# z619850002/CVIDS

Hardware: AMD Instinct MI355X
Metric: depth frames/sec integrated + Mvoxel-updates/sec, 640x480 @ 1 cm, 1/2/4/8 GPU (higher is better)
Workload: dtype f32; 1 GPU; 640x480 depth+BGR colour stream (sphere_room, 1 agent), 1 cm voxels, chunk 16^3, InverseTruncator(1), carving 0.05 m, projective TSDF integration + marching cubes every 10 frames; image=640x480, chunk=16, color=True, frames_per_call=10, mesh_every=10, parallelism=1 GPU

## Files before the change

cvids_amd/csrc/chisel_device.h:

```cpp
#pragma once
#include <hip/hip_runtime.h>
#include <stdint.h>

namespace chisel_hip {

constexpr uint64_t KEY_EMPTY = ~0ull;
constexpr uint64_t KEY_TOMB = ~0ull - 1ull;
constexpr int ID_BIAS = 1 << 20;
constexpr int INTEGRATE_MAX_GRID = 4096;
constexpr int INTEGRATE_GRID_CAP = 1 << 19;

__host__ __device__ inline uint64_t pack_id(int x, int y, int z) {
    return (uint64_t)(uint32_t)(x + ID_BIAS) | ((uint64_t)(uint32_t)(y + ID_BIAS) << 21) |
           ((uint64_t)(uint32_t)(z + ID_BIAS) << 42);
}
__host__ __device__ inline void unpack_id(uint64_t k, int &x, int &y, int &z) {
    x = (int)(k & 0x1FFFFF) - ID_BIAS;
    y = (int)((k >> 21) & 0x1FFFFF) - ID_BIAS;
    z = (int)((k >> 42) & 0x1FFFFF) - ID_BIAS;
}
__host__ __device__ inline uint64_t chunk_hash(int x, int y, int z) {
    return ((uint64_t)(int64_t)x * 73856093ull) ^ ((uint64_t)(int64_t)y * 19349663ull) ^
           ((uint64_t)(int64_t)z * 8349279ull);
}
// ... 32 lines not shown
    unsigned *mesh_flag;
    int *mesh_jobs;
    int *mesh_ctl;
    int mesh_jobs_capacity;
};

constexpr int MC_TRIS = 0, MC_GRIDS = 1, MC_OVERFLOW = 2, MC_JOBS = 3, MC_KEPT = 4, MC_CURSORS = 8;
constexpr int MC_BBOX = 136, MC_INTS = MC_BBOX + 8;
constexpr int MC_LATCH = 5;
__device__ inline void bbox_include(int *mesh_ctl, int x, int y, int z) {
    if (!mesh_ctl) return;
    int *b = mesh_ctl + MC_BBOX;
    if (x < b[0]) atomicMin(&b[0], x);
    if (y < b[1]) atomicMin(&b[1], y);
    if (z < b[2]) atomicMin(&b[2], z);
    if (x > b[3]) atomicMax(&b[3], x);
    if (y > b[4]) atomicMax(&b[4], y);
    if (z > b[5]) atomicMax(&b[5], z);
}

constexpr unsigned SUM_POS = 1u, SUM_NEG = 2u, SUM_ANY = 3u;
constexpr size_t SLOT_SUMMARY_PAD = 16;
__device__ inline uint32_t *slot_summary(const MapView &M) { return M.slot_dirty + 2 * (size_t)M.max_chunks + SLOT_SUMMARY_PAD; }

__device__ inline bool mark_slot_dirty(const MapView &M, int slot) {
    if (atomicExch(&M.slot_dirty[slot], 1u) == 0u) {
        const unsigned p = atomicAdd(&M.slot_dirty[2 * (size_t)M.max_chunks], 1u);
        if (p < (unsigned)M.max_chunks) M.slot_dirty[(size_t)M.max_chunks + p] = (unsigned)slot;
        return true;
    }
    return false;
}

constexpr int PYR_L0 = 2, PYR_L1 = 6, PYR_LEVELS = PYR_L1 - PYR_L0 + 1;
struct PyramidView {
    float2 *data;
    int off[PYR_LEVELS];
    int w[PYR_LEVELS];
    int h[PYR_LEVELS];
};

struct CameraParams {
    float R[9];
    float t[3];
    float fx, fy, cx, cy;
    int W, H;
};

constexpr int KMAX = 16;

struct IntegratorParams {
    int trunc_kind;
    float trunc_param;
    float weight;
    int carving;
    float carving_dist;
    float res;
    float half_res;
    float diag;
    float max_depth;
    int n_shards, shard_rank, shard_block;
    int single_chunk;
};

typedef float2 PixelRec;

// ... 184 lines not shown
```

cvids_amd/csrc/chisel_hip.hip:

```cpp
#include "../../include/chisel_hip.h"
#include "../../include/chisel_hip_selftest.h"

#include <hip/hip_runtime.h>
#include <hip/hip_ext.h>
#include <dlfcn.h>

#include <algorithm>
#include <array>
#include <atomic>
#include <chrono>
#include <condition_variable>
#include <functional>
#include <mutex>
#include <thread>
#include <cmath>
#include <cstdlib>
#include <cstdio>
#include <cstring>
#include <fstream>
#include <map>
#include <string>
#include <unordered_map>
#include <set>
#include <unordered_set>
// ... 235 lines not shown
    PinnedBuffer<int> mesh_totals_host;
    PinnedBuffer<int> error_flag_host;
    int mesh_seq = 0;
    PinnedBuffer<JobInfo> mesh_info_host;
    hipStream_t copy_stream = nullptr;
    ShellPlan shell_plan{};
    struct ShellMemory { DeviceBuffer<unsigned long long> jobset; DeviceBuffer<int> my_jobs, ctl, send_items; } shell_mem;
    PinnedBuffer<int> shell_plan_host;
    int64_t shell_send[SHELL_MAX_SHARDS][2] = {}, shell_recv[SHELL_MAX_SHARDS][2] = {};
    int shell_jobs = 0, shell_send_items = 0;
    const unsigned char *ghost_packed = nullptr;
    ShellSegments ghost_segments{};
    int ghost_packed_items = 0;
    hipEvent_t order_events[2] = {nullptr, nullptr};
    int64_t shell_stride = 0;
    unsigned shell_items_grid = 2048;
    const int *shell_abort_dev = nullptr;
    bool shell_fixed_ghosts = false, shell_redrop = false, shell_uncommitted = false;
    std::unordered_set<uint64_t, IdHash> pending_mesh_ids;
    uint64_t pending_version = 1;
    uint32_t dirty_epoch = 0;
    bool dirty_tail_queued = false;
    uint64_t dirty_tail_cursor = 0;
    unsigned dirty_tail_batch = 0;
    PinnedBuffer<int> dirty_tail_host;
    int batch_frames = KMAX;
    uint64_t ghost_bytes = 0;
    bool single_chunk = false;
    int single_id[3] = {0, 0, 0};
    bool mesh_mark_needed = false;
    bool mesh_totals_clean = true;
    int64_t removed_since_recompute = 0;
    int mesh_jobs_hint = 0;
    int mesh_stages = 3;
    bool mesh_detached = false;
    uint64_t topology_epoch = 0;
    MeshBuffers mesh_buf{};
    struct MeshMemory {
        DeviceBuffer<MeshJob> jobs; DeviceBuffer<int> ids; DeviceBuffer<JobInfo> info; DeviceBuffer<TriRec> tris; DeviceBuffer<CubeCorners> corners;
        DeviceBuffer<unsigned> cnt; DeviceBuffer<unsigned long long> job_acc; DeviceBuffer<double> query; DeviceBuffer<float> cube;
    } mesh_mem;
    struct CloudBuffers {
        DeviceBuffer<float> points, colors;
        int64_t capacity = 0;
        DeviceBuffer<char> zeroed;
        size_t zeroed_bytes = 0;
        CloudView view{};
        DeviceBuffer<CloudRay> rays; DeviceBuffer<unsigned> rgb; DeviceBuffer<int> tile_prefix, table_vals, pairs, sorted; DeviceBuffer<uint64_t> listed;
    } cloud;
    bool profiling = false;
    std::vector<ProfEvent> prof_live;
    std::vector<hipEvent_t> event_pool;
    double prof_ms[CHISEL_HIP_NUM_KERNELS] = {};
    int64_t prof_launches[CHISEL_HIP_NUM_KERNELS] = {};
};

namespace {

int sync_all(chisel_hip_map *m) {
    for (int pass = 0; pass < 2; pass++) {
        if (m->aux) HIP_TRY(hipStreamSynchronize(m->aux));
        if (m->aux2) HIP_TRY(hipStreamSynchronize(m->aux2));
        if (m->aux3) HIP_TRY(hipStreamSynchronize(m->aux3));
        if (!pass) HIP_TRY(hipStreamSynchronize(m->stream));
    }
    m->complete_seq = m->launch_seq;
// ... 2425 lines not shown
```

cvids_amd/csrc/host_mesh.h:

```cpp
namespace {

MeshParams mesh_params(const chisel_hip_map *m) {
    MeshParams P;
    P.res = m->cfg.voxel_resolution;
    P.half_res = m->cfg.voxel_resolution * 0.5f;
    P.rf_chunk = 1.0f / ((float)m->N * m->cfg.voxel_resolution);
    P.rf_voxel = 1.0f / m->cfg.voxel_resolution;
    P.use_color = m->cfg.use_color ? 1 : 0;
    P.stages = m->mesh_stages & m->tune.mesh_stage_mask;
    return P;
}

void launch_mesh_triangles(chisel_hip_map *m, const MeshParams &P, float *arena, size_t arena_floats, int publish = 0) {
    MeshBuffers &B = m->mesh_buf;
    const JobInfo *bases = B.info;
    const int *totals = B.totals;
    int *host_info = reinterpret_cast<int *>(m->mesh_info_host.dev());
    volatile int *host_flags = (volatile int *)m->mesh_totals_host.dev();
    const int max_jobs = std::min(MESH_INFO_PREFETCH, B.capacity), seq = m->mesh_seq, part = B.tri_capacity / MESH_PARTS;
    const dim3 grid(4096), block(MESH_TRI_BLOCK);
    switch (m->N) {
        case 8: hipLaunchKernelGGL(mesh_triangle_kernel<8>, grid, block, 0, m->stream, m->view, P, B.jobs, bases, B.tris, B.corners, totals, B.cnt, part, arena, arena_floats, host_info, host_flags, max_jobs, seq, publish); break;
        case 16: hipLaunchKernelGGL(mesh_triangle_kernel<16>, grid, block, 0, m->stream, m->view, P, B.jobs, bases, B.tris, B.corners, totals, B.cnt, part, arena, arena_floats, host_info, host_flags, max_jobs, seq, publish); break;
        case 32: hipLaunchKernelGGL(mesh_triangle_kernel<32>, grid, block, 0, m->stream, m->view, P, B.jobs, bases, B.tris, B.corners, totals, B.cnt, part, arena, arena_floats, host_info, host_flags, max_jobs, seq, publish); break;
    }
}

int mesh_subjobs(const chisel_hip_map *m) { return m->N == 8 ? MeshGeom<8>::S : (m->N == 16 ? MeshGeom<16>::S : MeshGeom<32>::S); }
int mesh_row_ints(const chisel_hip_map *m) { return m->N == 8 ? MeshGeom<8>::ROW : (m->N == 16 ? MeshGeom<16>::ROW : MeshGeom<32>::ROW); }
int ensure_mesh_jobs(chisel_hip_map *m, int n) {
    MeshBuffers &B = m->mesh_buf;
    if (n <= B.capacity) return CHISEL_HIP_OK;
    HIP_TRY(hipStreamSynchronize(m->stream));
    chisel_hip_map::MeshMemory &O = m->mesh_mem;
    int cap = std::max(4096, B.capacity);
    while (cap < n) cap *= 2;
    B.capacity = 0;
    HIP_TRY(alloc_viewed(O.jobs, B.jobs, (size_t)cap));
    HIP_TRY(alloc_viewed(O.ids, B.ids, (size_t)cap * 3));
    HIP_TRY(alloc_viewed(O.info, B.info, (size_t)cap));
    HIP_TRY(alloc_viewed(O.cnt, B.cnt, (size_t)cap * mesh_row_ints(m)));
    HIP_TRY(alloc_viewed(O.job_acc, B.job_acc, (size_t)cap));
    HIP_TRY(hipMemsetAsync(B.job_acc, 0, (size_t)cap * sizeof(unsigned long long), m->stream));
    B.capacity = cap;
    return CHISEL_HIP_OK;
}

enum { MT_TRIS = MC_TRIS, MT_GRIDS = MC_GRIDS, MT_OVERFLOW = MC_OVERFLOW, MT_JOBS = MC_JOBS };
int *mesh_totals(chisel_hip_map *m) { return m->mesh_buf.totals; }
hipError_t zero_mesh_counters(chisel_hip_map *m) {
    hipError_t e = hipMemsetAsync(mesh_totals(m), 0, 3 * sizeof(int), m->stream);
    if (e == hipSuccess) e = hipMemsetAsync(mesh_totals(m) + MC_CURSORS, 0, 2 * MESH_PARTS * sizeof(int), m->stream);
    return e;
// ... 107 lines not shown
        case 16: hipLaunchKernelGGL(mesh_count_kernel_16, grid, dim3(64), 0, m->stream, m->view, ids, ids_capacity, B.jobs, n_jobs, B.info, d_totals, B.cnt, B.job_acc, B.tris, B.corners, part, B.flags, keep, done_seq); break;
        case 32: hipLaunchKernelGGL(mesh_count_kernel_32, grid, dim3(64), 0, m->stream, m->view, ids, ids_capacity, B.jobs, n_jobs, B.info, d_totals, B.cnt, B.job_acc, B.tris, B.corners, part, B.flags, keep, done_seq); break;
    }
}

int recompute_meshes(chisel_hip_map *m) {
    RoctxRange range("chisel_hip mesh recompute: count, triangles");
    MeshBuffers &B = m->mesh_buf;
    const MeshParams P = mesh_params(m);
    if (!B.tris) {
        B.tri_capacity = std::max(B.tri_capacity, m->mesh_tiny ? 4 * MESH_PARTS : 1 << 20);
        HIP_TRY(alloc_viewed(m->mesh_mem.tris, B.tris, (size_t)B.tri_capacity));
        HIP_TRY(alloc_viewed(m->mesh_mem.corners, B.corners, (size_t)B.tri_capacity));
    }
    int arena_id = -1;
    for (size_t i = 0; i < m->arenas.size() && arena_id < 0; i++)
        if (!m->arenas[i].dev) arena_id = (int)i;
    if (arena_id < 0) {
        m->arenas.emplace_back();
        arena_id = (int)m->arenas.size() - 1;
    }
    {
        MeshArena &A = m->arenas[arena_id];
        A = MeshArena();
        int rc_a = take_arena_buffer(m, m->mesh_tiny ? (size_t)4096 : std::max<size_t>(2 * m->mesh_need_hint, (size_t)1 << 22), &A.dev, &A.capacity);
        if (rc_a) return rc_a;
    }
    launch_mesh_count(m);
    if (!m->mesh_detached) m->dirty_epoch++;
    m->mesh_seq++;
    m->recomputes++;
    {
        ProfScope ps(m, CHISEL_HIP_KERNEL_MESH);
        launch_mesh_triangles(m, P, m->arenas[arena_id].dev, m->arenas[arena_id].capacity, 1 | (B.n_jobs ? 2 : 0));
    }
    HIP_TRY(hipGetLastError());
    m->pending_meshes.unchecked = true;
    m->pending_meshes.active = false;
    m->pending_meshes.arena = arena_id;
    {
        const size_t want = std::max<size_t>(2 * m->mesh_need_hint, (size_t)1 << 22);
        bool have = false;
        for (const auto &b : m->arena_pool) have = have || b.second >= want;
        if (!have) {
            float *spare = nullptr;
            const size_t cap = want + want / 4 + 1024;
            if (hipMalloc(&spare, cap * sizeof(float)) == hipSuccess) m->arena_pool.emplace_back(spare, cap);
        }
    }
    return CHISEL_HIP_OK;
}

bool mesh_totals_published(const chisel_hip_map *m) { return ((volatile const int *)m->mesh_totals_host.get())[MH_PUBLISHED] == m->mesh_seq; }
int replay_deferred_set(chisel_hip_map *m, int set);
void launch_fixed_drop(chisel_hip_map *m, const int *latch);
int check_mesh_totals(chisel_hip_map *m) {
    if (!m->pending_meshes.unchecked) return CHISEL_HIP_OK;
    m->pending_meshes.unchecked = false;
    const int deferred = m->deferred_set;
    m->deferred_set = -1;
    MeshBuffers &B = m->mesh_buf;
    int *d_totals = mesh_totals(m);
    const bool color = m->cfg.use_color != 0;
    const MeshParams P = mesh_params(m);
    int arena_id = m->pending_meshes.arena;
    {
        volatile int *host = m->mesh_totals_host.get();
// ... 42 lines not shown
                HIP_TRY(hipMemcpyAsync(B.n_jobs, stage, sizeof(int), hipMemcpyHostToDevice, m->stream));
            }
            launch_mesh_count(m);
            if (B.n_jobs) HIP_TRY(hipMemsetAsync(B.n_jobs, 0, sizeof(int), m->stream));
            HIP_TRY(hipMemcpyAsync(totals, d_totals, 4 * sizeof(int), hipMemcpyDeviceToHost, m->stream));
            HIP_TRY(hipStreamSynchronize(m->stream));
            if (!totals[MT_OVERFLOW]) break;
            if (attempt == 12) return fail(CHISEL_HIP_ERR_HIP, "mesh record lists overflow after growing them");
        }
        redo = true;
        HIP_TRY(hipMemcpy(m->mesh_info_host.get(), B.info, (size_t)std::min(MESH_INFO_PREFETCH, B.capacity) * sizeof(JobInfo), hipMemcpyDeviceToHost));
    }
    const int n = totals[MT_JOBS];
    if ((size_t)totals[MT_TRIS] > 0x7fffffffull / 9) return fail(CHISEL_HIP_ERR_UNSUPPORTED, "more than 2^31 / 9 mesh triangles in one recompute");
    const size_t nv = (size_t)totals[MT_TRIS] * 3, ng = (size_t)totals[MT_GRIDS];
    {
        MeshArena &A = m->arenas[arena_id];
        A.nv = nv;
        A.ng = ng;
        A.color = color;
        if (redo ? !device_unfit : (A.floats() > A.capacity) != device_unfit)
            return fail(CHISEL_HIP_ERR_HIP, "mesh recompute: host and device disagree on whether it fitted");
        if (redo || A.floats() > A.capacity) {
            HIP_TRY(hipStreamSynchronize(m->stream));
            HIP_TRY(hipMemsetAsync(mesh_totals(m) + MC_LATCH, 0, sizeof(int), m->stream));
            if (A.floats() > A.capacity) {
                m->arena_pool.emplace_back(A.dev, A.capacity);
                A.dev = nullptr;
                int rc_a = take_arena_buffer(m, A.floats(), &A.dev, &A.capacity);
                if (rc_a) return rc_a;
            }
            {
                ProfScope ps(m, CHISEL_HIP_KERNEL_MESH);
                launch_mesh_triangles(m, P, A.dev, A.capacity);
            }
            HIP_TRY(hipGetLastError());
            latch_guard.settled = true;
            if (m->shell_redrop && m->ghost_packed)
                launch_fixed_drop(m, nullptr);
            if (deferred >= 0) {
                int rc_r = replay_deferred_set(m, deferred);
                if (rc_r) return rc_r;
            }
        }
        m->mesh_need_hint = A.floats();
        if (nv + ng == 0) {
            free_arena(m, A);
            arena_id = -1;
        }
    }
    if (m->shell_redrop) {
        m->shell_redrop = false;
        m->ghost_packed = nullptr;
    }
    m->mesh_jobs_hint = n;
    if (n != 0) {
        m->pending_meshes.active = true;
        m->pending_meshes.n = n;
        m->pending_meshes.arena = arena_id;
    }
    if (pool_error != 0)
        return fail(CHISEL_HIP_ERR_POOL_FULL, pool_error == 1 ? "chunk pool exhausted: raise chisel_hip_config.max_chunks"
                                                              : "chunk hash table exhausted: raise chisel_hip_config.max_chunks");
    return CHISEL_HIP_OK;
}

int resolve_pending_meshes(chisel_hip_map *m) {
    int rc_c = check_mesh_totals(m);
    if (rc_c) return rc_c;
    if (!m->pending_meshes.active) return CHISEL_HIP_OK;
    m->pending_meshes.active = false;
    MeshBuffers &B = m->mesh_buf;
    const int n = m->pending_meshes.n, arena_id = m->pending_meshes.arena;
    {
        volatile int *host = m->mesh_totals_host.get();
        const auto t0 = std::chrono::steady_clock::now();
        while (host[MH_INFO_SEQ] != m->mesh_seq) {
            if (std::chrono::steady_clock::now() - t0 > std::chrono::milliseconds(2)) {
                HIP_TRY(hipStreamSynchronize(m->stream));
                if (host[MH_INFO_SEQ] != m->mesh_seq) return fail(CHISEL_HIP_ERR_HIP, "mesh job records were not published");
            }
        }
        std::atomic_thread_fence(std::memory_order_acquire);
    }
    g_mesh_timer.lap(1);
    std::vector<JobInfo> tail;
    if (n > MESH_INFO_PREFETCH) {
        tail.resize((size_t)n - MESH_INFO_PREFETCH);
// ... 467 lines not shown
```

cvids_amd/csrc/kernels_integrate.h:

```cpp
#pragma once
#include <type_traits>

#include "chisel_device.h"
#include "kernels_cull.h"
#include "kernels_map.h"

namespace chisel_hip {

#ifndef INTEGRATE_WAVES
#define INTEGRATE_WAVES 6
#endif
#ifndef INTEGRATE_BLOCKS_PER_CU
#define INTEGRATE_BLOCKS_PER_CU 6
#endif
#ifndef INTEGRATE_WPB
#define INTEGRATE_WPB 1
#endif
#ifndef INTEGRATE_FINE_BELOW
#define INTEGRATE_FINE_BELOW 600
#endif

#ifndef INTEGRATE_PIPE
#define INTEGRATE_PIPE 0
#endif
// ... 550 lines not shown
            if (!existed) {
                if (bm) {
                    int s = 0;
                    if (lane == 0) s = claim_slot(Mc, sy, cxi, cyi, czi);
                    s = __builtin_amdgcn_readfirstlane(s);
                    const bool created = s >= 0 && (s & CLAIM_CREATED) != 0;
                    slot = s >= 0 ? (s & ~CLAIM_CREATED) : s;
                    n_new += created ? 1u : 0u;
                }
                unsigned seen = 0u;
                if (lane == 0 && bm) seen += atomicOr(&sy->band, bm);
                if (lane < KMAX && carve_v) seen += atomicAdd(&sy->carve[lane], (unsigned)carve_v);
                asm volatile("s_waitcnt vmcnt(0)" : "+v"(seen)::"memory");
                unsigned last = 0u;
                if (lane == 0) last = (atomicAdd(&sy->arrived, 1u) == (unsigned)(G::WPC - 1)) ? 1u : 0u;
                if (__builtin_amdgcn_readfirstlane((int)last)) {
                    unsigned band_all = 0u, cnt = 0u;
                    if (lane == 0) band_all = atomicOr(&sy->band, 0u);
                    if (lane < KMAX) cnt = atomicAdd(&sy->carve[lane], 0u);
                    band_all = (unsigned)__builtin_amdgcn_readfirstlane((int)band_all);
                    const bool counts = band_all != 0u && lane < KMAX && lane > __builtin_ctz(band_all | 0x80000000u);
                    unsigned v = counts ? cnt : 0u;
#pragma unroll
                    for (int o = 8; o > 0; o >>= 1) v += __shfl_down(v, o);
                    if (lane == 0) t_probe += v;
                }
                PHASE(2);
                if (slot < 0) return;
            }
            unsigned signs = 0u;
            {
                const size_t out_base = (size_t)slot * G::V;
                if (st & DCHG) {
                    *reinterpret_cast<QuadF *>((M.sdf + out_base) + lane_off) = s4;
                    *reinterpret_cast<QuadF *>((M.wgt + out_base) + lane_off) = w4;
                }
                if (COLOR && (st & CCHG)) *reinterpret_cast<QuadU *>((M.rgbw + out_base) + lane_off) = c4;
                bool pos = false, neg = false;
#pragma unroll
                for (int j = 0; j < VPL; j++) {
                    const bool seen = (st & DCHG) && f4(w4, j) > 0.5f;
                    neg = neg || (seen && f4(s4, j) < 0.0f);
                    pos = pos || (seen && !(f4(s4, j) < 0.0f));
                }
                signs = (__any(pos) ? SUM_POS : 0u) | (__any(neg) ? SUM_NEG : 0u);
            }
            if (cm) {
                unsigned old = 0u;
                int newly_dirty = 0;
                if (lane == 0) {
                    old = atomicOr(&sy->changed, cm);
                    if (old == 0u) newly_dirty = mark_slot_dirty(M, slot) ? 1 : 0;
                    if (signs) atomicOr(&slot_summary(M)[slot], signs);
                }
                old = (unsigned)__builtin_amdgcn_readfirstlane((int)old);
                n_updated += (unsigned)__popc(cm & ~old);
                if (__builtin_amdgcn_readfirstlane(newly_dirty)) mesh_expand_dirty(Mc, slot, cxi, cyi, czi, lane);
            }
    };
    if (mixed) {
        if (local_unit < units_x) {
            const int u4 = n_coarse_x * G::WPC;
            if (local_unit < u4) run_unit(std::integral_constant<int, VPL0>{}, (local_unit / G::WPC) * 8 + xcd, local_unit % G::WPC, local_unit);
            else run_unit(std::integral_constant<int, 2>{}, (n_coarse_x + (local_unit - u4) / GF::WPC) * 8 + xcd, (local_unit - u4) % GF::WPC, local_unit);
        }
        PHASE(3);
    }
    int wid = mixed ? total : ((local_unit / G::WPC) * 8 + xcd) * G::WPC + local_unit % G::WPC;
    while (wid < total) {
        run_unit(std::integral_constant<int, VPL0>{}, wid / G::WPC, wid % G::WPC, wid);
// ... 94 lines not shown
```

cvids_amd/csrc/kernels_mesh.h:

```cpp
#pragma once
#include "chisel_device.h"
#include "kernels_map.h"
#include "mc_tables.h"

namespace chisel_hip {

__constant__ unsigned long long c_mc_cases[256] = CHISEL_MC_PACKED_CASES;
__constant__ __attribute__((aligned(4))) unsigned char c_mc_counts[256] = CHISEL_MC_VERTEX_COUNTS;
__constant__ unsigned char c_mc_edges[12] = CHISEL_MC_EDGE_CORNERS;

struct MeshJob {
    int x, y, z;
    int nb[27];
    int pad[2];
};
constexpr int NB_SELF = 13;

struct MeshParams {
    float res;
    float half_res;
    float rf_chunk;
    float rf_voxel;
    int use_color;
    int stages;
// ... 225 lines not shown
__device__ inline float fold_corner(float sdf, float weight) { return weight > 0.5f ? sdf : __builtin_nanf(""); }

template <int N>
struct MeshGeom {
    static constexpr int ZL = N == 16 ? 2 : (N == 8 ? 7 : 1);
    static constexpr int NI = (N - 1 + ZL - 1) / ZL;
    static constexpr int S = NI + 3;
    static constexpr int CPL = N == 32 ? 16 : 8;
    static constexpr int MAXC = 64 * CPL;
    static constexpr int TILE = N == 32 ? 33 * 33 * 2 : N * N * (ZL + 1);
    static constexpr int ROW = (2 + S + 3) / 4 * 4;
    static_assert((N - 1) * (N - 1) * ZL <= MAXC && N * N <= MAXC, "cubes per sub-job");
};
template <int N, int TYPE>
struct MeshBox {
    static constexpr int BX = TYPE == 1 ? 1 : (TYPE == 3 ? N : N - 1);
    static constexpr int BY = TYPE == 2 ? 1 : (TYPE == 0 ? N - 1 : N);
    static constexpr int TX = BX + 1, TY = BY + 1;
    static constexpr int X0 = TYPE == 1 ? N - 1 : 0, Y0 = TYPE == 2 ? N - 1 : 0;
    static constexpr unsigned PLUS = TYPE == 0 ? 0x01u : (TYPE == 1 ? 0x0Fu : (TYPE == 2 ? 0x05u : 0xFFu));
};
constexpr int MESH_PARTS = 64;
static_assert(MC_BBOX == MC_CURSORS + 2 * MESH_PARTS, "the created-id box sits behind the cursors");
static_assert(MC_LATCH > MC_KEPT && MC_LATCH < MC_CURSORS, "a free word in front of the cursors");
static_assert(MESH_PARTS == 64, "integrate_kernel zeroes the cursors with one wave");

#ifndef MESH_COUNT_WAVES
#define MESH_COUNT_WAVES 6
#endif
#ifndef MESH_COUNT_VGPRS
#define MESH_COUNT_VGPRS 80
#endif
constexpr int MESH_TRI_BLOCK = 256;
#ifndef MESH_TRI_WAVES
#define MESH_TRI_WAVES 1
#endif

struct JobInfo {
    int x, y, z;
    int present;
    int n_vertices, n_grids;
    int tri_base;
    int grid_base;
};

struct alignas(16) TriRec {
    unsigned job;
    unsigned code;
    unsigned cube;
    unsigned rel;
};
struct alignas(16) CubeCorners {
    float s[8];
};
__device__ inline float pick8(const float (&s)[8], int e) {
    const float a0 = (e & 1) ? s[1] : s[0], a1 = (e & 1) ? s[3] : s[2], a2 = (e & 1) ? s[5] : s[4], a3 = (e & 1) ? s[7] : s[6];
    const float b0 = (e & 2) ? a1 : a0, b1 = (e & 2) ? a3 : a2;
    return (e & 4) ? b1 : b0;
}

#ifdef CHISEL_PHASES
__device__ unsigned long long g_mesh_phase[8];
#define MSTAMP(i) do { if (lane == 0 && (blockIdx.x & 31) == 0) { const unsigned long long n_ = __builtin_amdgcn_s_memrealtime(); atomicAdd(&g_mesh_phase[i], n_ - mt_); mt_ = n_; } } while (0)
#else
#define MSTAMP(i) do { } while (0)
#endif
// ... 33 lines not shown
#endif
        __syncthreads();
        asm volatile("" : "+v"(lane));
        const int jx = ids[3 * j], jy = ids[3 * j + 1], jz = ids[3 * j + 2];
        const int type = s < G::NI ? 0 : s - G::NI + 1;
        const unsigned plus_needed = type == 0 ? MeshBox<N, 0>::PLUS : (type == 1 ? MeshBox<N, 1>::PLUS : (type == 2 ? MeshBox<N, 2>::PLUS : MeshBox<N, 3>::PLUS));
        const int dx = lane % 3 - 1, dy = (lane / 3) % 3 - 1, dz = lane / 9 - 1;
        const bool plus = lane < 27 && dx >= 0 && dy >= 0 && dz >= 0;
        const bool counted = plus && ((plus_needed >> (dx + 2 * dy + 4 * dz)) & 1u);
        int slot = -1;
        unsigned sum = 0u;
        if (lane < 27 && (s == 0 || counted)) slot = hash_find_quiescent(M, jx + dx, jy + dy, jz + dz);
        if (counted && slot >= 0) sum = slot_summary(M)[slot];
        if (lane < 27) s_nb[lane] = slot;
        if (s == 0) {
            if (lane < 27) jobs[j].nb[lane] = slot;
            else if (lane == 27) {
                jobs[j].x = jx;
                jobs[j].y = jy;
                jobs[j].z = jz;
                jobs[j].pad[0] = jobs[j].pad[1] = 0;
            }
        }
        const int self = __shfl(slot, NB_SELF);
        const bool present = self >= 0;
        const bool can = present && (unsigned)__shfl((int)sum, NB_SELF) != 0u && __ballot(counted && (sum & SUM_POS)) != 0ull && __ballot(counted && (sum & SUM_NEG)) != 0ull;
        if (s == 0 && lane == 28 && present && !keep_dirty) {
            if (mesh_flag) mesh_flag[self] = 0u;
            M.slot_dirty[self] = 0u;
        }
        MSTAMP(0);
        auto deposit = [&](int my_nt, int my_ng, int part) -> unsigned long long {
            unsigned long long old = 0ull;
            if (lane == 1) cnt[(size_t)j * G::ROW + 2 + s] = (unsigned)my_nt | ((unsigned)my_ng << 16);
            if (lane == 1 || (lane == 0 && my_ng)) {
                unsigned long long *addr = lane == 0 ? cursors + part : job_acc + j;
                const unsigned long long inc = lane == 0 ? ((unsigned long long)my_ng << 32) | (unsigned long long)my_nt
                                                         : (1ull << 48) | ((unsigned long long)my_ng << 24) | (unsigned long long)my_nt;
                old = atomicAdd(addr, inc);
                if (lane == 1 && (int)(old >> 48) == G::S - 1) {
                    const unsigned long long tot = old + inc;
                    const int tnt = (int)(tot & 0xffffffull), tng = (int)((tot >> 24) & 0xffffffull);
                    unsigned long long base = 0ull;
                    if (tnt | tng) base = atomicAdd(reinterpret_cast<unsigned long long *>(ctl + MC_TRIS), ((unsigned long long)tng << 32) | (unsigned long long)tnt);
                    JobInfo ji;
                    ji.x = jx; ji.y = jy; ji.z = jz;
                    ji.present = present ? 1 : 0;
                    ji.n_vertices = 3 * tnt;
                    ji.n_grids = tng;
                    ji.tri_base = (int)(base & 0xffffffffull);
                    ji.grid_base = (int)(base >> 32);
                    info[j] = ji;
                    cnt[(size_t)j * G::ROW] = (unsigned)ji.tri_base;
                    cnt[(size_t)j * G::ROW + 1] = (unsigned)ji.grid_base;
                    job_acc[j] = 0ull;
                }
            }
            return old;
        };
        if (!can) {
            (void)deposit(0, 0, 0);
            continue;
        }
        auto run = [&](auto type_tag) {
            constexpr int T = decltype(type_tag)::value;
            using B = MeshBox<N, T>;
            const int z0 = T == 0 ? s * G::ZL : (T == 3 ? N - 1 : 0);
            const int bz = T == 0 ? min(G::ZL, N - 1 - z0) : (T == 3 ? 1 : N - 1);
            const int ncubes = B::BX * B::BY * bz;
            if (T == 0) {
                constexpr int PASS = N == 32 ? 4 : ((G::ZL + 1) * N * N / 4 + 63) / 64;
                const int n4 = (bz + 1) * N * N / 4;
                const float4 *sp = reinterpret_cast<const float4 *>(M.sdf + (size_t)self * (N * N * N) + (size_t)z0 * N * N);
                const float4 *wp = reinterpret_cast<const float4 *>(M.wgt + (size_t)self * (N * N * N) + (size_t)z0 * N * N);
                for (int base = 0; base < n4; base += 64 * PASS) {
                    float4 vs[PASS], vw[PASS];
#pragma unroll
                    for (int u = 0; u < PASS; u++) {
                        const int i = min(base + u * 64 + lane, n4 - 1);
                        vs[u] = sp[i];
                        vw[u] = wp[i];
                    }
#pragma unroll
                    for (int u = 0; u < PASS; u++) {
                        const int i = base + u * 64 + lane;
                        if (i < n4)
                            reinterpret_cast<float4 *>(s_tile)[i] = make_float4(fold_corner(vs[u].x, vw[u].x), fold_corner(vs[u].y, vw[u].y),
// ... 69 lines not shown
            }
            const int tv = __shfl(iv, 63), tg = __shfl(ig, 63);
            MSTAMP(3);
            const int part = (j * G::S + s) & (MESH_PARTS - 1);
            const unsigned long long old = deposit(tv / 3, tg, part);
            if (tg == 0) return;
            const unsigned long long cur = (unsigned long long)__shfl((long long)old, 0);
            const int cur_t = (int)(cur & 0xffffffffull), cur_g = (int)(cur >> 32);
            MSTAMP(4);
            if (cur_t + tv / 3 > part_capacity || cur_g + tg > part_capacity) {
                if (lane == 0) ctl[MC_OVERFLOW] = 1;
                return;
            }
            {
                int trel = (iv - nv) / 3, gidx = ig - ng;
#pragma unroll
                for (int k = 0; k < G::CPL; k++) {
                    const int c = lane * G::CPL + k;
                    const int index = (c < ncubes) ? (int)((cw[k >> 2] >> ((k & 3) * 8)) & 0xffu) : 0;
                    if (index == 0) continue;
                    s_list[gidx] = (unsigned)c | ((unsigned)index << 10) | ((unsigned)trel << 18);
                    trel += n_verts(index) / 3;
                    gidx++;
                }
            }
            __syncthreads();
            const size_t base_t = (size_t)part * part_capacity + cur_t, base_g = (size_t)part * part_capacity + cur_g;
            for (int e = lane; e < tg; e += 64) {
                const unsigned a = s_list[e];
                const int c = (int)(a & 1023u), index = (int)((a >> 10) & 255u), trel = (int)(a >> 18);
                CubeCorners cc;
                int idx2;
                (void)cube_corners(c, cc.s, idx2);
                corners[base_g + e] = cc;
                const int x = B::X0 + c % B::BX, y = B::Y0 + (c / B::BX) % B::BY, z = z0 + c / (B::BX * B::BY);
                const int nt = n_verts(index) / 3;
                TriRec rec;
                rec.job = (unsigned)j;
                rec.cube = (unsigned)(base_g + e);
                for (int t = 0; t < nt; t++) {
                    rec.code = (unsigned)x | ((unsigned)y << 5) | ((unsigned)z << 10) | ((unsigned)index << 15) | ((unsigned)t << 23) | ((unsigned)s << 26);
                    rec.rel = (unsigned)(trel + t) | ((unsigned)e << 16);
                    tris[base_t + trel + t] = rec;
                }
            }
            MSTAMP(5);
        };
        switch (type) {
            case 0: run(std::integral_constant<int, 0>()); break;
            case 1: run(std::integral_constant<int, 1>()); break;
            case 2: run(std::integral_constant<int, 2>()); break;
            default: run(std::integral_constant<int, 3>()); break;
        }
    }
}

#define CHISEL_MESH_COUNT_KERNEL(NN, VGPRS, WAVES)                                                                                                    \
    __global__ __launch_bounds__(64, WAVES) __attribute__((amdgpu_num_vgpr(VGPRS))) void mesh_count_kernel_##NN(                                 \
        MapView M, const int *__restrict__ ids, int ids_capacity, MeshJob *jobs, const int *__restrict__ n_jobs, JobInfo *info, int *ctl, unsigned *cnt, \
        unsigned long long *job_acc, TriRec *tris, CubeCorners *corners, int part_capacity, unsigned *mesh_flag, int keep_dirty, int done_seq) { \
        mesh_count_body<NN>(M, ids, ids_capacity, jobs, n_jobs, info, ctl, cnt, job_acc, tris, corners, part_capacity, mesh_flag, keep_dirty, done_seq); \
    }
CHISEL_MESH_COUNT_KERNEL(8, MESH_COUNT_VGPRS, MESH_COUNT_WAVES)
CHISEL_MESH_COUNT_KERNEL(16, MESH_COUNT_VGPRS, MESH_COUNT_WAVES)
CHISEL_MESH_COUNT_KERNEL(32, 128, 3)
#undef CHISEL_MESH_COUNT_KERNEL

__device__ inline f3v interpolate_vertex(f3v v1, f3v v2, float sdf1, float sdf2) {
    const float minDiff = 1e-6;
    const float sdfDiff = sdf1 - sdf2;
    if (fabsf(sdfDiff) < minDiff) return add3(v1, scl3(v2, 0.5f));
    const float t = sdf1 / sdfDiff;
    return add3(v1, scl3(sub3(v2, v1), t));
}

__device__ inline int corner_ox(int i) { return ((i + 1) >> 1) & 1; }
// ... 61 lines not shown
        if (s_off[part + o] <= i) part += o;
    i -= s_off[part];
    TSTAMP(0, i);
    const TriRec rec = tris[(size_t)part * part_capacity + i];
    const MeshJob &job = jobs[rec.job];
    const int *nb = job.nb;
    const int jx = job.x, jy = job.y, jz = job.z;
    const int x = (int)(rec.code & 31u), y = (int)((rec.code >> 5) & 31u), z = (int)((rec.code >> 10) & 31u);
    const int index = (int)((rec.code >> 15) & 0xffu), t = 3 * (int)((rec.code >> 23) & 7u), sub = (int)(rec.code >> 26);
    int tri_pos = (int)(rec.rel & 0xffffu), grid_pos = (int)(rec.rel >> 16);
    {
        const uint4 *row4 = reinterpret_cast<const uint4 *>(cnt + (size_t)rec.job * ROW);
        uint4 r[ROW / 4];
#pragma unroll
        for (int q = 0; q < ROW / 4; q++) r[q] = row4[q];
        tri_pos += (int)r[0].x;
        grid_pos += (int)r[0].y;
#pragma unroll
        for (int q = 2; q < ROW; q++) {
            const unsigned c = (q & 3) == 0 ? r[q >> 2].x : ((q & 3) == 1 ? r[q >> 2].y : ((q & 3) == 2 ? r[q >> 2].z : r[q >> 2].w));
            const unsigned cc = (q - 2 < sub) ? c : 0u;
            tri_pos += (int)(cc & 0xffffu);
            grid_pos += (int)(cc >> 16);
        }
    }
    const int vi = 3 * tri_pos + mine;
    TSTAMP(1, vi);
    const unsigned long long row = c_mc_cases[index];
    const f3v origin = mk3((float)(N * jx) * P.res, (float)(N * jy) * P.res, (float)(N * jz) * P.res);
    const f3v coords = add3(mk3((float)x * P.res + P.half_res, (float)y * P.res + P.half_res, (float)z * P.res + P.half_res), origin);
    const CubeCorners cc = corners[rec.cube];
    if (t == 0 && mine == 0) {
        const size_t g = (size_t)grid_pos;
        grids[3 * g] = coords.x;
        grids[3 * g + 1] = coords.y;
        grids[3 * g + 2] = coords.z;
    }
    f3v p[3];
#pragma unroll
    for (int a = 0; a < 3; a++) {
        const int ed = (int)((row >> (4 * (t + 2 - a))) & 0xF);
        const int e0 = c_mc_edges[ed] & 0xF, e1 = c_mc_edges[ed] >> 4;
        const f3v c0 = add3(coords, mk3((float)corner_ox(e0) * P.res, (float)corner_oy(e0) * P.res, (float)corner_oz(e0) * P.res));
        const f3v c1 = add3(coords, mk3((float)corner_ox(e1) * P.res, (float)corner_oy(e1) * P.res, (float)corner_oz(e1) * P.res));
        const float s0 = pick8(cc.s, e0), s1 = pick8(cc.s, e1);
        p[a] = interpolate_vertex(c0, c1, s0, s1);
    }
    const f3v fn = normalized3(cross3v(sub3(p[1], p[0]), sub3(p[2], p[0])));
    const f3v pv = mine == 0 ? p[0] : (mine == 1 ? p[1] : p[2]);
    float *vo = vertices + 3 * (size_t)vi;
    float *no = normals + 3 * (size_t)vi;
    vo[0] = pv.x;
    vo[1] = pv.y;
    vo[2] = pv.z;
    TSTAMP(2, pv.x);
    f3v nrm = fn;
    double dist;
    f3v grad;
    if ((P.stages & 1) && get_sdf_and_gradient<N>(M, P, pv, jx, jy, jz, nb, dist, grad)) {
        const float mag = sqrtf(sum3f(grad.x * grad.x, grad.y * grad.y, grad.z * grad.z));
        if ((double)mag > 1e-12) nrm = scl3(grad, 1.0f / mag);
    }
    TSTAMP(3, nrm.x);
    no[0] = nrm.x;
    no[1] = nrm.y;
    no[2] = nrm.z;
    if (colors) {
        const f3v col = (P.stages & 2) ? interpolate_color<N>(M, P, pv, jx, jy, jz, nb) : mk3(0.0f, 0.0f, 0.0f);
        float *co = colors + 3 * (size_t)vi;
        TSTAMP(4, col.x);
        co[0] = col.x;
        co[1] = col.y;
        co[2] = col.z;
    }
    }
    }
}

template <int N>
__global__ void mesh_one_cube_kernel(MapView M, MeshParams P, int jx, int jy, int jz, int ix, int iy, int iz, float cx, float cy, float cz, float *out) {
    float sdf[8];
    bool observed = true;
    for (int i = 0; i < 8 && observed; i++) {
        int c[3] = {ix + corner_ox(i), iy + corner_oy(i), iz + corner_oz(i)};
        int off[3] = {0, 0, 0};
        for (int a = 0; a < 3; a++) {
            if (c[a] < 0) { off[a] = -1; c[a] = N - 1; }
            else if (c[a] >= N) { off[a] = 1; c[a] = 0; }
        }
        const int slot = hash_find_quiescent(M, jx + off[0], jy + off[1], jz + off[2]);
        if (slot < 0) { observed = false; break; }
        const size_t o = (size_t)slot * (N * N * N) + (c[2] * N + c[1]) * N + c[0];
        if (!(M.wgt[o] > 0.5f)) { observed = false; break; }
        sdf[i] = M.sdf[o];
    }
    out[0] = 0.0f;
    out[1] = 0.0f;
    if (!observed) return;
    int index = 0;
    for (int i = 0; i < 8; i++) index |= (sdf[i] < 0.0f) ? (1 << i) : 0;
    const int nv = c_mc_counts[index];
    const unsigned long long row = c_mc_cases[index];
    const f3v coords = mk3(cx, cy, cz);
    for (int t = 0; t < nv; t += 3) {
        f3v p[3];
        for (int a = 0; a < 3; a++) {
// ... 121 lines not shown
```

Measured before the change: 106,800 frames/s.

## Size mesh triangle grid from triangle hint and compute face normals lazily

Launches the mesh triangle kernel with a grid sized from the previous triangle count, instead of a fixed 4096 blocks, clamped between 64 and 4096. The per-vertex kernel now interpolates only its own edge vertex and computes the full face normal only when the SDF gradient is unavailable. Store sites are routed through a templated store_out helper that can emit nontemporal or relaxed atomic stores, but every mode defaults to a plain store. The aim is to cut idle blocks and redundant vertex interpolation. A stale hint could undersize the grid, which is only safe if the kernel grid-strides over its work.

```diff
diff --git a/cvids_amd/csrc/chisel_device.h b/cvids_amd/csrc/chisel_device.h
--- a/cvids_amd/csrc/chisel_device.h
+++ b/cvids_amd/csrc/chisel_device.h
@@ -88,6 +88,52 @@
     return false;
 }
 
+#ifndef MESH_TRI_STORE
+#define MESH_TRI_STORE 0
+#endif
+#ifndef INTEGRATE_STORE
+#define INTEGRATE_STORE 0
+#endif
+#ifndef MESH_COUNT_STORE
+#define MESH_COUNT_STORE 0
+#endif
+typedef unsigned out_u2 __attribute__((ext_vector_type(2)));
+typedef unsigned out_u4 __attribute__((ext_vector_type(4)));
+template <int MODE, typename T>
+__device__ __forceinline__ void store_out(T *p, const T &v) {
+    static_assert(sizeof(T) == 4 || sizeof(T) == 8 || sizeof(T) == 16 || sizeof(T) == 32, "store_out: 4, 8, 16 or 32 bytes");
+    if constexpr (MODE == 0) {
+        *p = v;
+    } else if constexpr (MODE == 2) {
+        if constexpr (sizeof(T) == 4) {
+            unsigned w;
+            __builtin_memcpy(&w, &v, 4);
+            __builtin_nontemporal_store(w, reinterpret_cast<unsigned *>(p));
+        } else if constexpr (sizeof(T) == 8) {
+            out_u2 w;
+            __builtin_memcpy(&w, &v, 8);
+            __builtin_nontemporal_store(w, reinterpret_cast<out_u2 *>(p));
+        } else {
+            out_u4 w[sizeof(T) / 16];
+            __builtin_memcpy(w, &v, sizeof(T));
+#pragma unroll
+            for (int i = 0; i < (int)(sizeof(T) / 16); i++) __builtin_nontemporal_store(w[i], reinterpret_cast<out_u4 *>(p) + i);
+        }
+    } else {
+        if constexpr (sizeof(T) == 4) {
+            unsigned w;
+            __builtin_memcpy(&w, &v, 4);
+            __hip_atomic_store(reinterpret_cast<unsigned *>(p), w, __ATOMIC_RELAXED, __HIP_MEMORY_SCOPE_AGENT);
+        } else {
+            unsigned long long w[sizeof(T) / 8];
+            __builtin_memcpy(w, &v, sizeof(T));
+#pragma unroll
+            for (int i = 0; i < (int)(sizeof(T) / 8); i++)
+                __hip_atomic_store(reinterpret_cast<unsigned long long *>(p) + i, w[i], __ATOMIC_RELAXED, __HIP_MEMORY_SCOPE_AGENT);
+        }
+    }
+}
+
 constexpr int PYR_L0 = 2, PYR_L1 = 6, PYR_LEVELS = PYR_L1 - PYR_L0 + 1;
 struct PyramidView {
     float2 *data;
diff --git a/cvids_amd/csrc/chisel_hip.hip b/cvids_amd/csrc/chisel_hip.hip
--- a/cvids_amd/csrc/chisel_hip.hip
+++ b/cvids_amd/csrc/chisel_hip.hip
@@ -291,6 +291,7 @@
     bool mesh_totals_clean = true;
     int64_t removed_since_recompute = 0;
     int mesh_jobs_hint = 0;
+    int mesh_tris_hint = 0;
     int mesh_stages = 3;
     bool mesh_detached = false;
     uint64_t topology_epoch = 0;
diff --git a/cvids_amd/csrc/host_mesh.h b/cvids_amd/csrc/host_mesh.h
--- a/cvids_amd/csrc/host_mesh.h
+++ b/cvids_amd/csrc/host_mesh.h
@@ -11,14 +11,19 @@
     return P;
 }
 
-void launch_mesh_triangles(chisel_hip_map *m, const MeshParams &P, float *arena, size_t arena_floats, int publish = 0) {
+void launch_mesh_triangles(chisel_hip_map *m, const MeshParams &P, float *arena, size_t arena_floats, int publish = 0, long long tris_hint = 0) {
     MeshBuffers &B = m->mesh_buf;
     const JobInfo *bases = B.info;
     const int *totals = B.totals;
     int *host_info = reinterpret_cast<int *>(m->mesh_info_host.dev());
     volatile int *host_flags = (volatile int *)m->mesh_totals_host.dev();
     const int max_jobs = std::min(MESH_INFO_PREFETCH, B.capacity), seq = m->mesh_seq, part = B.tri_capacity / MESH_PARTS;
-    const dim3 grid(4096), block(MESH_TRI_BLOCK);
+#if MESH_TRI_GRID_SIZED
+    const long long want = tris_hint > 0 ? (3 * (tris_hint + tris_hint / 4) + MESH_TRI_BLOCK - 1) / MESH_TRI_BLOCK : 4096;
+#else
+    const long long want = 4096;
+#endif
+    const dim3 grid((unsigned)std::min<long long>(std::max<long long>(want, 64), 4096)), block(MESH_TRI_BLOCK);
     switch (m->N) {
         case 8: hipLaunchKernelGGL(mesh_triangle_kernel<8>, grid, block, 0, m->stream, m->view, P, B.jobs, bases, B.tris, B.corners, totals, B.cnt, part, arena, arena_floats, host_info, host_flags, max_jobs, seq, publish); break;
         case 16: hipLaunchKernelGGL(mesh_triangle_kernel<16>, grid, block, 0, m->stream, m->view, P, B.jobs, bases, B.tris, B.corners, totals, B.cnt, part, arena, arena_floats, host_info, host_flags, max_jobs, seq, publish); break;
@@ -192,7 +197,7 @@
     m->recomputes++;
     {
         ProfScope ps(m, CHISEL_HIP_KERNEL_MESH);
-        launch_mesh_triangles(m, P, m->arenas[arena_id].dev, m->arenas[arena_id].capacity, 1 | (B.n_jobs ? 2 : 0));
+        launch_mesh_triangles(m, P, m->arenas[arena_id].dev, m->arenas[arena_id].capacity, 1 | (B.n_jobs ? 2 : 0), m->mesh_tris_hint);
     }
     HIP_TRY(hipGetLastError());
     m->pending_meshes.unchecked = true;
@@ -301,7 +306,7 @@
             }
             {
                 ProfScope ps(m, CHISEL_HIP_KERNEL_MESH);
-                launch_mesh_triangles(m, P, A.dev, A.capacity);
+                launch_mesh_triangles(m, P, A.dev, A.capacity, 0, totals[MT_TRIS]);
             }
             HIP_TRY(hipGetLastError());
             latch_guard.settled = true;
@@ -323,6 +328,7 @@
         m->ghost_packed = nullptr;
     }
     m->mesh_jobs_hint = n;
+    m->mesh_tris_hint = totals[MT_TRIS];
     if (n != 0) {
         m->pending_meshes.active = true;
         m->pending_meshes.n = n;
diff --git a/cvids_amd/csrc/kernels_integrate.h b/cvids_amd/csrc/kernels_integrate.h
--- a/cvids_amd/csrc/kernels_integrate.h
+++ b/cvids_amd/csrc/kernels_integrate.h
@@ -606,10 +606,10 @@
             {
                 const size_t out_base = (size_t)slot * G::V;
                 if (st & DCHG) {
-                    *reinterpret_cast<QuadF *>((M.sdf + out_base) + lane_off) = s4;
-                    *reinterpret_cast<QuadF *>((M.wgt + out_base) + lane_off) = w4;
-                }
-                if (COLOR && (st & CCHG)) *reinterpret_cast<QuadU *>((M.rgbw + out_base) + lane_off) = c4;
+                    store_out<INTEGRATE_STORE>(reinterpret_cast<QuadF *>((M.sdf + out_base) + lane_off), s4);
+                    store_out<INTEGRATE_STORE>(reinterpret_cast<QuadF *>((M.wgt + out_base) + lane_off), w4);
+                }
+                if (COLOR && (st & CCHG)) store_out<INTEGRATE_STORE>(reinterpret_cast<QuadU *>((M.rgbw + out_base) + lane_off), c4);
                 bool pos = false, neg = false;
 #pragma unroll
                 for (int j = 0; j < VPL; j++) {
diff --git a/cvids_amd/csrc/kernels_mesh.h b/cvids_amd/csrc/kernels_mesh.h
--- a/cvids_amd/csrc/kernels_mesh.h
+++ b/cvids_amd/csrc/kernels_mesh.h
@@ -281,6 +281,9 @@
 #define MESH_COUNT_VGPRS 80
 #endif
 constexpr int MESH_TRI_BLOCK = 256;
+#ifndef MESH_TRI_GRID_SIZED
+#define MESH_TRI_GRID_SIZED 1
+#endif
 #ifndef MESH_TRI_WAVES
 #define MESH_TRI_WAVES 1
 #endif
@@ -380,7 +383,7 @@
         MSTAMP(0);
         auto deposit = [&](int my_nt, int my_ng, int part) -> unsigned long long {
             unsigned long long old = 0ull;
-            if (lane == 1) cnt[(size_t)j * G::ROW + 2 + s] = (unsigned)my_nt | ((unsigned)my_ng << 16);
+            if (lane == 1) store_out<MESH_COUNT_STORE>(&cnt[(size_t)j * G::ROW + 2 + s], (unsigned)my_nt | ((unsigned)my_ng << 16));
             if (lane == 1 || (lane == 0 && my_ng)) {
                 unsigned long long *addr = lane == 0 ? cursors + part : job_acc + j;
                 const unsigned long long inc = lane == 0 ? ((unsigned long long)my_ng << 32) | (unsigned long long)my_nt
@@ -398,9 +401,9 @@
                     ji.n_grids = tng;
                     ji.tri_base = (int)(base & 0xffffffffull);
                     ji.grid_base = (int)(base >> 32);
-                    info[j] = ji;
-                    cnt[(size_t)j * G::ROW] = (unsigned)ji.tri_base;
-                    cnt[(size_t)j * G::ROW + 1] = (unsigned)ji.grid_base;
+                    store_out<MESH_COUNT_STORE>(&info[j], ji);
+                    store_out<MESH_COUNT_STORE>(&cnt[(size_t)j * G::ROW], (unsigned)ji.tri_base);
+                    store_out<MESH_COUNT_STORE>(&cnt[(size_t)j * G::ROW + 1], (unsigned)ji.grid_base);
                     job_acc[j] = 0ull;
                 }
             }
@@ -536,7 +539,7 @@
                 CubeCorners cc;
                 int idx2;
                 (void)cube_corners(c, cc.s, idx2);
-                corners[base_g + e] = cc;
+                store_out<MESH_COUNT_STORE>(&corners[base_g + e], cc);
                 const int x = B::X0 + c % B::BX, y = B::Y0 + (c / B::BX) % B::BY, z = z0 + c / (B::BX * B::BY);
                 const int nt = n_verts(index) / 3;
                 TriRec rec;
@@ -545,7 +548,7 @@
                 for (int t = 0; t < nt; t++) {
                     rec.code = (unsigned)x | ((unsigned)y << 5) | ((unsigned)z << 10) | ((unsigned)index << 15) | ((unsigned)t << 23) | ((unsigned)s << 26);
                     rec.rel = (unsigned)(trel + t) | ((unsigned)e << 16);
-                    tris[base_t + trel + t] = rec;
+                    store_out<MESH_COUNT_STORE>(&tris[base_t + trel + t], rec);
                 }
             }
             MSTAMP(5);
@@ -673,46 +676,51 @@
     const CubeCorners cc = corners[rec.cube];
     if (t == 0 && mine == 0) {
         const size_t g = (size_t)grid_pos;
-        grids[3 * g] = coords.x;
-        grids[3 * g + 1] = coords.y;
-        grids[3 * g + 2] = coords.z;
-    }
-    f3v p[3];
-#pragma unroll
-    for (int a = 0; a < 3; a++) {
+        store_out<MESH_TRI_STORE>(&grids[3 * g], coords.x);
+        store_out<MESH_TRI_STORE>(&grids[3 * g + 1], coords.y);
+        store_out<MESH_TRI_STORE>(&grids[3 * g + 2], coords.z);
+    }
+    auto edge_vertex = [&](int a) -> f3v {
         const int ed = (int)((row >> (4 * (t + 2 - a))) & 0xF);
         const int e0 = c_mc_edges[ed] & 0xF, e1 = c_mc_edges[ed] >> 4;
         const f3v c0 = add3(coords, mk3((float)corner_ox(e0) * P.res, (float)corner_oy(e0) * P.res, (float)corner_oz(e0) * P.res));
         const f3v c1 = add3(coords, mk3((float)corner_ox(e1) * P.res, (float)corner_oy(e1) * P.res, (float)corner_oz(e1) * P.res));
         const float s0 = pick8(cc.s, e0), s1 = pick8(cc.s, e1);
-        p[a] = interpolate_vertex(c0, c1, s0, s1);
-    }
-    const f3v fn = normalized3(cross3v(sub3(p[1], p[0]), sub3(p[2], p[0])));
-    const f3v pv = mine == 0 ? p[0] : (mine == 1 ? p[1] : p[2]);
+        return interpolate_vertex(c0, c1, s0, s1);
+    };
+    const f3v pv = edge_vertex(mine);
     float *vo = vertices + 3 * (size_t)vi;
     float *no = normals + 3 * (size_t)vi;
-    vo[0] = pv.x;
-    vo[1] = pv.y;
-    vo[2] = pv.z;
+    store_out<MESH_TRI_STORE>(&vo[0], pv.x);
+    store_out<MESH_TRI_STORE>(&vo[1], pv.y);
+    store_out<MESH_TRI_STORE>(&vo[2], pv.z);
     TSTAMP(2, pv.x);
-    f3v nrm = fn;
+    f3v nrm = mk3(0.0f, 0.0f, 0.0f);
+    bool shaded = false;
     double dist;
     f3v grad;
     if ((P.stages & 1) && get_sdf_and_gradient<N>(M, P, pv, jx, jy, jz, nb, dist, grad)) {
         const float mag = sqrtf(sum3f(grad.x * grad.x, grad.y * grad.y, grad.z * grad.z));
-        if ((double)mag > 1e-12) nrm = scl3(grad, 1.0f / mag);
+        if ((double)mag > 1e-12) {
+            nrm = scl3(grad, 1.0f / mag);
+            shaded = true;
+        }
+    }
+    if (!shaded) {
+        const f3v p0 = edge_vertex(0), p1 = edge_vertex(1), p2 = edge_vertex(2);
+        nrm = normalized3(cross3v(sub3(p1, p0), sub3(p2, p0)));
     }
     TSTAMP(3, nrm.x);
-    no[0] = nrm.x;
-    no[1] = nrm.y;
-    no[2] = nrm.z;
+    store_out<MESH_TRI_STORE>(&no[0], nrm.x);
+    store_out<MESH_TRI_STORE>(&no[1], nrm.y);
+    store_out<MESH_TRI_STORE>(&no[2], nrm.z);
     if (colors) {
         const f3v col = (P.stages & 2) ? interpolate_color<N>(M, P, pv, jx, jy, jz, nb) : mk3(0.0f, 0.0f, 0.0f);
         float *co = colors + 3 * (size_t)vi;
         TSTAMP(4, col.x);
-        co[0] = col.x;
-        co[1] = col.y;
-        co[2] = col.z;
+        store_out<MESH_TRI_STORE>(&co[0], col.x);
+        store_out<MESH_TRI_STORE>(&co[1], col.y);
+        store_out<MESH_TRI_STORE>(&co[2], col.z);
     }
     }
     }
```

Result: slower. 102,600 frames/s (-3.9%).
